# mhozza/covest

Measured on AMD Instinct MI355X. Metric: grid-point log-likelihood evals/s, repeat model, 10k-bin hist, higher is better.
Workload: dtype f64

## Files before the change

### covest_amd/csrc/ll_factored.hip

```cpp
#include <hip/hip_runtime.h>

#include <algorithm>
#include <mutex>
#include <type_traits>

#include "direct_point.h"
#include "handback.h"
#include "fastmath.h"
#include "kernels.h"
#include "point_fetch.h"
#include "streams.h"
#include "wave.h"

namespace covest {

namespace {

typedef double d4 __attribute__((ext_vector_type(4)));

constexpr double kShareScale = 0x1p128;


template <int N, int MU>
__device__ __forceinline__ void contract_step(int i, const double *cur, const int (&a_off)[MU], const int (&cut)[MU],
                                              const double (&r4)[MU], double (&wrun)[MU], d4 (&acc)[MU])
{
    double a[N];
#pragma unroll
    for (int k = 0; k < N; ++k)
        a[k] = cur[a_off[k] + 4 * i];
#pragma unroll
    for (int k = 0; k < N; ++k) {
        const double w = (i < cut[k]) ? wrun[k] : 0.0;
        wrun[k] *= r4[k];
        acc[k] = __builtin_amdgcn_mfma_f64_16x16x4f64(a[k], w, acc[k], 0, 0, 0);
    }
}

[[maybe_unused]] constexpr int kLdWide = 290;
template <int NT, int HU, bool TAIL, bool PLAIN, int LDC = 0>
__global__ __launch_bounds__(NT) void ll_factored_kernel(const DevModel m, const int32_t n_tiles, const int32_t n_items,
                                                         const double *__restrict__ tile_dbl,
                                                         const int32_t *__restrict__ tile_int,
                                                         const FactoredPlan plan,
                                                         double *__restrict__ out_ll, const SubList sub_list)
{
    const TileView tv = tile_view_from(n_tiles, n_items, tile_dbl, tile_int);
#ifdef COVEST_DIAG
    const long long dgx_0 = (long long)clock64();
    long long dgx_1 = 0, dgx_2 = 0, dgx_3 = 0, dgx_4 = 0;
#endif
    constexpr int NW = NT / kWave;
    constexpr int MU = 2 * HU;
    static_assert(MU == 6, "contract loops are written for 6 slots");
    constexpr bool SPO = PLAIN && TAIL;
    constexpr bool NEED_SCAL = !PLAIN;
    constexpr int LOG_DEG = PLAIN ? 3 : 5;
    const int LD = LDC ? LDC : plan.ld;
    constexpr int NE = FactoredLds::entries_of(NT);
    const FactoredLds lay{NT, plan.n_buf, LD, SPO};
    extern __shared__ double Gs[];
    __shared__ __attribute__((aligned(16))) double log_tab[kLogTableDoubles];
    __shared__ unsigned sub_rec[NE * 2];
    __shared__ __attribute__((aligned(16))) double2 rowc[2][kTileBins];
    __shared__ __attribute__((aligned(16))) double rows[NEED_SCAL ? 2 : 1][NEED_SCAL ? kTileBins : 2];
    __shared__ __attribute__((aligned(16))) double rho_tab[PLAIN ? NW * MU * 4 : 4];
    __shared__ double lconst_s;
    static_assert(MU == kMaxUnits, "the LDS layout counts kMaxUnits slots a wave");
    static_assert(sizeof(log_tab) + sizeof(sub_rec) + sizeof(rowc) + sizeof(rows) + sizeof(rho_tab) + sizeof(lconst_s) + 6 * 15 <=
                      kFactoredStaticLds, "the planners' LDS budget (tiles.h) must hold the kernel's static LDS");

    const int tid = threadIdx.x;
    const int lane = tid & (kWave - 1);
    const int wave = __builtin_amdgcn_readfirstlane(tid / kWave);
    const double p_clamp = plan.p_clamp;
    const double zero_frac = kZeroSteps * (kGridStep / p_clamp);
    const int list_mode = PLAIN ? 0 : plan.list_mode;

    const int n_seg = list_mode ? plan.n_seg : 1;
    const int unit = list_mode ? (int)blockIdx.x / n_seg : (int)blockIdx.x;
    const int seg = list_mode ? (int)blockIdx.x - unit * n_seg : 0;
    const int seg_items = (n_items + n_seg - 1) / n_seg;
    const int t_begin = seg * seg_items, t_end = min(n_items, t_begin + seg_items);
    const int64_t ce = (PLAIN || list_mode == 0) ? plan.ce_end - 1 - unit : plan.ce_begin + unit;
    const bool list = list_mode == 1 || list_mode == 2;
    const int64_t ic = list ? ce : ce / plan.n_e;
    const int64_t ie = list ? ce : ce - ic * plan.n_e;
    double par[kMaxParams] = {plan.c_axis[ic], plan.e_axis[ie], 0, 0, 0};
    constexpr int kLogPerThread = (kLogTableDoubles + NT - 1) / NT;
    double log_v[kLogPerThread];
#pragma unroll
    for (int u = 0; u < kLogPerThread; ++u)
        log_v[u] = kLogTable[min(tid + u * NT, kLogTableDoubles - 1)];
    const double rho_v = PLAIN ? plan.unit_rho[(int64_t)blockIdx.y * NW * MU * 4 + min(tid, NW * MU * 4 - 1)] : 0.0;
    double lc_first = 0.0;
    if (wave == NW - 1 && t_begin + lane < t_end)
        lc_first = tv.item_lconst[t_begin + lane];
#pragma unroll
    for (int u = 0; u < kLogPerThread; ++u)
        if (tid + u * NT < kLogTableDoubles)
            log_tab[tid + u * NT] = log_v[u];
    if (PLAIN && tid < NW * MU * 4)
        rho_tab[tid] = rho_v;
#pragma unroll
    for (int u = 0; u < (NE + NT - 1) / NT; ++u)
        if (tid + u * NT < NE) {
            sub_rec[2 * (tid + u * NT)] = 0xFFFFFFFFu;
            sub_rec[2 * (tid + u * NT) + 1] = 0;
        }
    clamp_point<2>(m, par);
    const bool finite = isfinite(par[0]) && isfinite(par[1]);
    const int n_pass = PLAIN ? 1 : plan.n_pass;
    if (tid < 8 * n_pass)
        Gs[lay.rates() + tid] = error_class_rate_mul(m, par[0], par[1], tid, m.n_err);
    if (wave == NW - 1) {
        double lc = 0.0 + lc_first;
        for (int t = t_begin + lane + kWave; t < t_end; t += kWave)
            lc += tv.item_lconst[t];
        lc = wave_sum(lc);
        if (lane == 0)
            lconst_s = PLAIN ? lc - kLogRawBias<kScaleBits> * tv.suf_h[0] : lc;
    }
    __syncthreads();
#ifdef COVEST_DIAG
    dgx_1 = (long long)clock64();
#endif

    const int my_pass = n_pass == 1 ? 0 : tid / plan.pass_stride;
    const int o_local = n_pass == 1 ? tid : tid - my_pass * plan.pass_stride;
    const bool wave_builds = wave * kWave < plan.n_columns;
    const int o_base = PLAIN ? 0 : list_mode == 2 ? plan.item_obase[ce] : plan.o_base;
    const int o_mine = o_base + o_local + 1;
    double lam[8];
#pragma unroll
    for (int s = 0; s < 8; ++s)
        lam[s] = Gs[lay.rates() + 8 * my_pass + s];
    double n_total = -1.0;
    if (n_pass > 1) {
        n_total = 0.0;
        for (int s = 0; s < 8 * n_pass; ++s)
            n_total += m.comb[s] * (1.0 - exp_neg_rn((double)o_mine * Gs[lay.rates() + s]));
    }
    __syncthreads();
    StreamSet<8> st;
    if (wave_builds) {
        st.template init<false>(m, lam, o_mine, finite && my_pass < n_pass && o_local < plan.max_o, log_tab,
                                log_tab, 8 * my_pass, n_total);
    } else {
        st.gone = 0u;
#pragma unroll
        for (int s = 0; s < 8; ++s) {
            st.v[s] = 0.0;
            st.x[s] = 0.0;
            st.an.set(s, 0.0, -INFINITY);
        }
    }
#ifdef COVEST_DIAG
    dgx_2 = (long long)clock64();
#endif
    const bool lane_in_row = tid < LD - 2;
    if (tid < FactoredLds::kSlack)
        Gs[lay.slack() + tid] = 0.0;
    if (tid < lay.rows()) {
        Gs[lay.pad(tid)] = 0.0;
        Gs[lay.pad(tid) + 1] = 0.0;
    }

    const int col = lane & 15;
    const int kq = lane >> 4;
    int len[MU], cont[MU], uhalf[MU], qslot[MU], cut[MU], a_off0[MU], nsh[MU];
    double r4[MU], llacc[MU];
    uint64_t dead[MU];
    unsigned off_slots = 0;
    bool newly_dead = false;
    CompSum spacc[(TAIL && !SPO) ? MU : 1];
    CompSum so = {0.0, 0.0};
    auto wave_block = [&](int w) -> int {
        if (list)
            return w >= NW - 2 ? 1 + 2 * (int)ce + (w - (NW - 2)) : 0;
        return (int)blockIdx.y * NW + w;
    };
    const int slot_base = wave_block(wave) * MU;
    int u_qt[MU], u_s0[MU], u_len[MU], u_cont[MU], u_half[MU], u_nsh[MU], u_o0[MU], u_T[MU];
#pragma unroll
    for (int k = 0; k < MU; ++k) {
        const int at = slot_base + k;
        u_qt[k] = plan.unit_tile[at];
        u_s0[k] = plan.unit_s0[at];
        u_len[k] = plan.unit_len[at];
        u_cont[k] = plan.unit_cont[at];
        u_half[k] = plan.unit_half[at];
        u_nsh[k] = PLAIN ? plan.unit_nsh[at] : 0;
        u_o0[k] = plan.unit_o0[at];
    }
#pragma unroll
    for (int k = 0; k < MU; ++k) {
        const int qt = __builtin_amdgcn_readfirstlane(u_qt[k]);
        const bool on = qt >= 0;
        const int slot = (on ? qt : 0) * 16 + col;
        qslot[k] = on ? slot : -1;
        u_T[k] = plan.q_T[slot];
        r4[k] = plan.q_r4[slot];
    }
#pragma unroll
    for (int k = 0; k < MU; ++k) {
        const bool on = qslot[k] >= 0;
        const int first_step = __builtin_amdgcn_readfirstlane(u_s0[k]);
        len[k] = __builtin_amdgcn_readfirstlane(u_len[k]);
        cont[k] = __builtin_amdgcn_readfirstlane(u_cont[k]);
        uhalf[k] = __builtin_amdgcn_readfirstlane(u_half[k]);
        nsh[k] = PLAIN ? __builtin_amdgcn_readfirstlane(u_nsh[k]) : 0;
        a_off0[k] = (16 * uhalf[k] + col) * LD + kq + 4 * first_step;
        const int t_lane = on ? u_T[k] : 0;
        const int o0 = __builtin_amdgcn_readfirstlane(u_o0[k]);
        cut[k] = ((t_lane - (o0 + kq) + 3) >> 2) - nsh[k];
        llacc[k] = 0.0;
        dead[k] = 0;
        spacc[(TAIL && !SPO) ? k : 0].hi = 0.0;
        spacc[(TAIL && !SPO) ? k : 0].lo = 0.0;
    }

    unsigned m_first = 0, m_cont = 0, m_sh = 0;
#pragma unroll
    for (int k = 0; k < MU; ++k) {
        m_first |= (qslot[k] >= 0 && !cont[k]) ? 1u << k : 0u;
        m_cont |= cont[k] ? 1u << k : 0u;
        m_sh |= nsh[k] > 0 ? 1u << k : 0u;
    }
    double wfirst[MU], wrun[MU];
    auto load_weights = [&]() {
#pragma unroll
        for (int k = 0; k < MU; ++k) {
            const double2 pw = reinterpret_cast<const double2 *>(plan.piece_w)[(int64_t)(slot_base + k) * kWave + lane];
            wfirst[k] = pw.x;
            wrun[k] = pw.y;
        }
    };
    load_weights();

    long long dg_a = 0, dg_b = 0, dg_b0 = 0, dg_c = 0, dg_w = 0, dg_t0 = 0, dg_zero = 0, dg_enter = 0, dg_first = 0;
#ifdef COVEST_DIAG
    const bool diag = plan.diag != nullptr;
#else
    constexpr bool diag = false;
#endif
    auto walk_tile = [&](auto n_tag, double *colp, double renorm, double k0) __attribute__((always_inline)) -> double {
        constexpr int N = decltype(n_tag)::value;
        if (!lane_in_row)
            return 0.0;
        double xx[8];
#pragma unroll
        for (int s = 0; s < 8; ++s) {
            double xs = st.x[s];
            if (s < N) {
                asm volatile("" : "+v"(xs));
                xx[s] = xs * xs;
            } else {
                xx[s] = 0.0;
            }
        }
        double *row = colp;
        double tsum = 0.0;
        if (SPO) {
            double kk = k0;
#pragma unroll
            for (int b = 0; b < kTileBins; b += 2) {
                double g1, g2;
                st.template step2n<N>(xx, g1, g2);
                row[0] = g1;
                row[LD] = g2;
                row += 2 * LD;
                tsum = fma(tsum, kk, g1);
                kk += 1.0;
                tsum = fma(tsum, kk, g2);
                kk += 1.0;
            }
            tsum *= renorm;
        } else {
#pragma unroll
            for (int b = 0; b < kTileBins; b += 2) {
                double g1, g2;
                st.template step2n<N>(xx, g1, g2);
                row[0] = g1;
                row[LD] = g2;
                row += 2 * LD;
            }
        }
        st.template leave_tile_n<N>(renorm);
        return tsum;
    };
    auto build_tile = [&](int t, bool seg_start, double *dst) __attribute__((always_inline)) -> double {
        if (COVEST_SKIP_PHASE(plan, 1))
            return 0.0;
        const TileRec rc = tv.rec[t];
        const double k0 = rc.k0;
        const int nb = rc.nb;
        const int n_live = st.enter_tile(k0 - 1.0, k0 + (double)(nb - 1), rc.lgam_prev, rc.lgam_last,
                                         rc.run_start != 0 || seg_start);
        if (diag) {
            const long long now__ = (long long)clock64();
            dg_enter += now__ - dg_t0;
            dg_t0 = now__;
        }
        double *colp = dst + (lane_in_row ? tid : 0);
        const double *scal = tv.scal + (int64_t)t * kTileBins;
        if (nb == kTileBins && !(SPO && rc.has_filler != 0)) {
            if (n_live > 4)
                return walk_tile(std::integral_constant<int, 8>{}, colp, rc.renorm, k0);
            if (n_live > 2)
                return walk_tile(std::integral_constant<int, 4>{}, colp, rc.renorm, k0);
            if (n_live == 2)
                return walk_tile(std::integral_constant<int, 2>{}, colp, rc.renorm, k0);
            if (n_live == 1)
                return walk_tile(std::integral_constant<int, 1>{}, colp, rc.renorm, k0);
            if (lane_in_row) {
                if (diag)
                    dg_zero += 1;
#pragma unroll
                for (int b = 0; b < kTileBins; ++b)
                    colp[b * LD] = 0.0;
            }
            return 0.0;
        }
        double tsum = 0.0;
        for (int b = 0; b < kTileBins; ++b) {
            const double g = b < nb ? st.step() : 0.0;
            if (SPO && b < nb)
                tsum = fma(g, scal[b], tsum);
            if (lane_in_row)
                colp[b * LD] = g;
        }
        st.leave_tile(rc.renorm);
        return tsum * 0x1p476;
    };
    auto sum_tile = [&](auto n_tag, const double *scal_ptr, double scal_or_k0, double renorm) __attribute__((always_inline)) -> double {
        constexpr int N = decltype(n_tag)::value;
        double xx[8];
#pragma unroll
        for (int s = 0; s < 8; ++s) {
            double xs = st.x[s];
            if (s < N) {
                asm volatile("" : "+v"(xs));
                xx[s] = xs * xs;
            } else {
                xx[s] = 0.0;
            }
        }
        double gsum = 0.0;
        if (SPO) {
            double kk = scal_or_k0;
#pragma unroll
            for (int b = 0; b < kTileBins; b += 2) {
                double g1, g2;
                st.template step2n<N>(xx, g1, g2);
                gsum = fma(gsum, kk, g1);
                kk += 1.0;
                gsum = fma(gsum, kk, g2);
                kk += 1.0;
            }
            st.template leave_tile_n<N>(renorm);
            return gsum * renorm;
        }
        const double *scal = SPO ? nullptr : scal_ptr;
#pragma unroll
        for (int half = 0; half < 2; ++half) {
            double sc[16];
#pragma unroll
            for (int b = 0; b < 16; ++b)
                sc[b] = scal[16 * half + b];
            asm volatile("" ::: "memory");
#pragma unroll
            for (int b = 0; b < 16; b += 2) {
                double g1, g2;
                st.template step2n<N>(xx, g1, g2);
                gsum = fma(g1, sc[b], gsum);
                gsum = fma(g2, sc[b + 1], gsum);
            }
        }
        st.template leave_tile_n<N>(renorm);
        return gsum * (1.0 / kBasicScale);
    };
    auto build_tile_sum = [&](int t, bool seg_start) __attribute__((always_inline)) -> double {
        const TileRec rc = tv.rec[t];
        const double k0 = rc.k0;
        const int nb = rc.nb;
        const int n_live = SPO ? st.enter_sum_tile(k0 - 1.0, k0 + (double)(nb - 1), rc.lgam_prev, rc.lgam_last,
                                                   rc.run_start != 0 || seg_start)
                               : st.enter_tile(k0 - 1.0, k0 + (double)(nb - 1), rc.lgam_prev, rc.lgam_last,
                                               rc.run_start != 0 || seg_start);
        const double *scal = tv.scal + (int64_t)t * kTileBins;
        if (nb == kTileBins && !(SPO && rc.has_filler != 0)) {
            if (n_live > 2)
                return sum_tile(std::integral_constant<int, 8>{}, scal, k0, rc.renorm);
            if (n_live == 2)
                return sum_tile(std::integral_constant<int, 2>{}, scal, k0, rc.renorm);
            if (n_live == 1)
                return sum_tile(std::integral_constant<int, 1>{}, scal, k0, rc.renorm);
            return 0.0;
        }
        double gsum = 0.0;
        for (int b = 0; b < nb; ++b)
            gsum = fma(st.step(), scal[b], gsum);
        st.leave_tile(rc.renorm);
        return SPO ? gsum * 0x1p476 : gsum * (1.0 / kBasicScale);
    };
    bool resync = false;
    auto build_item = [&](int it, bool seg_start, double *dst) __attribute__((always_inline)) {
        const int first = TAIL ? __builtin_amdgcn_readfirstlane(tv.item_first[it]) : it;
        if (TAIL && tv.item_sum[it] != 0) {
            if (COVEST_SKIP_PHASE(plan, 1))
                return;
            const int n = __builtin_amdgcn_readfirstlane(tv.item_ntiles[it]);
            if (SPO) {
                if (!seg_start) {
                    const int tl = first + n - 1;
                    const TileRec ra = tv.rec[first], rb = tv.rec[tl];
                    const double ka = ra.k0 - 1.0, kb = rb.k0 + (double)(rb.nb - 1);
                    const double lga = ra.lgam_prev, lgb = rb.lgam_last;
                    bool matters = false;
#pragma unroll
                    for (int s = 0; s < 8; ++s) {
                        if ((st.gone >> s) & 1u)
                            continue;
                        const double lx = st.an.lx(s), c = st.an.c(s);
                        const double top = fmax(fma(ka, lx, c - lga), fma(kb, lx, c - lgb));
                        matters = matters || !(top < StreamSet<8>::kSumWindowLn) || (st.x[s] >= ka - 1.0 && st.x[s] <= kb + 1.0);
                    }
                    if (!__any(matters)) {
#pragma unroll
                        for (int s = 0; s < 8; ++s)
                            st.v[s] = 0.0;
                        resync = true;
                        return;
                    }
                }
                for (int r = 0; r < n; ++r) {
                    if (st.gone == 0xFFu && !(seg_start && r == 0))
                        break;
                    so.add(build_tile_sum(first + r, (seg_start && r == 0) || resync));
                    resync = false;
                }
                return;
            }
            double *colp = dst + (lane_in_row ? tid : 0);
            for (int r = 0; r < n; ++r) {
                const double gsum = build_tile_sum(first + r, seg_start && r == 0);
                if (lane_in_row)
                    colp[r * LD] = gsum;
            }
            for (int r = n; r < kTileBins; ++r)
                if (lane_in_row)
                    colp[r * LD] = 0.0;
        } else {
            const double tsum = build_tile(first, seg_start || (SPO && resync), dst);
            resync = false;
            if (SPO)
                so.add(tsum);
        }
    };

#define STAMP(acc)                                    \
    if (diag) {                                       \
        const long long now__ = (long long)clock64(); \
        acc += now__ - dg_t0;                         \
        dg_t0 = now__;                                \
    }
    if (diag)
        dg_t0 = (long long)clock64();
#ifdef COVEST_DIAG
    dgx_3 = (long long)clock64();
#endif

    const bool dbuf = plan.n_buf == 2;
    double nxt_h = 0.0, nxt_c = 0.0, nxt_s = 0.0;
    auto fetch_rows = [&](int it) {
        if (tid < kTileBins && it < t_end) {
            const int64_t at = (int64_t)it * kTileBins + tid;
            nxt_h = tv.item_cnt[at];
            nxt_c = tv.item_iscal[at];
            if (NEED_SCAL)
                nxt_s = tv.item_scal[at];
        }
    };
    int last_item = t_end - 1;
    if (SPO)
        while (last_item > t_begin && tv.item_sum[last_item] != 0)
            --last_item;
    const bool last_first = PLAIN && t_end - t_begin >= 2 && last_item > t_begin;
    auto tile_at = [&](int p) -> int { return last_first ? (p == t_begin ? last_item : (p <= last_item ? p - 1 : p)) : p; };
    const int t_endx = t_end + (SPO ? 1 : 0);
    fetch_rows(tile_at(t_begin));
    for (int p = t_begin - (dbuf ? 1 : 0); p < t_endx; ++p) {
        const int pb = dbuf ? p + 1 : p;
        if (SPO && pb == t_end) {
            if (wave_builds && lane_in_row) {
                double *dst = Gs + lay.buf(pb) + tid;
                dst[0] = so.hi * 0x1p-540;
                dst[LD] = so.lo * 0x1p-540;
            }
        } else if (pb < t_end) {
            if (tid < kTileBins) {
                rowc[pb & 1][tid] = make_double2(nxt_h, p_clamp * nxt_c);
                if (NEED_SCAL)
                    rows[pb & 1][tid] = nxt_s;
            }
            fetch_rows(pb + 1 < t_end ? tile_at(pb + 1) : t_end);
            if (wave_builds) {
                if (last_first && pb == t_begin + 1)
                    st.gone = 0u;
                build_item(tile_at(pb), pb == t_begin || (last_first && (pb == t_begin + 1 || pb == last_item + 1)),
                           Gs + lay.buf(pb));
            }
        }
        STAMP(dg_a)
        if (!dbuf)
            __syncthreads();
        const bool sp_item = SPO && p == t_end;
        if (p >= t_begin && !(SPO && !sp_item && tv.item_sum[tile_at(p)] != 0)) {
            const int t = tile_at(p);
            const double *cur = Gs + lay.buf(p);
            d4 acc[MU];
            const d4 zero4 = (d4){0.0, 0.0, 0.0, 0.0};
            double a0[MU];
#pragma unroll
            for (int k = 0; k < MU; ++k)
                a0[k] = cur[a_off0[k]];
            if (diag) {
                double sink = 0.0;
#pragma unroll
                for (int k = 0; k < MU; ++k)
                    sink += a0[k] + wfirst[k];
                asm volatile("" ::"v"(sink));
                const long long now__ = (long long)clock64();
                dg_first += now__ - dg_t0;
                dg_t0 = now__;
            }
#pragma unroll
            for (int k = 0; k < MU; ++k) {
                if (!PLAIN || !((m_sh >> k) & 1u) || COVEST_SKIP_PHASE(plan, 8)) {
                    acc[k] = len[k] > 0 ? __builtin_amdgcn_mfma_f64_16x16x4f64(a0[k], wfirst[k], zero4, 0, 0, 0) : zero4;
                    continue;
                }
                const double rr16 = rho_tab[4 * (wave * MU + k)];
                const double2 rt = *reinterpret_cast<const double2 *>(&rho_tab[4 * (wave * MU + k) + 2]);
                const double rr4 = rt.x, rho_n = rt.y;
                const double *g1 = cur + a_off0[k];
                int nsh_k = nsh[k];
                asm volatile("" : "+s"(nsh_k));
                const int n4 = nsh_k >> 2, rem = nsh_k & 3;
                const double *top = g1 + 4 * (1 + 4 * n4);
                const double *zp = Gs + FactoredLds{NT, plan.n_buf, LD, SPO}.slack();
                double h0 = *(rem > 0 ? top : zp), h1 = *(rem > 1 ? top + 4 : zp), h2 = *(rem > 2 ? top + 8 : zp), h3 = 0.0;
                {
                    unsigned qa = (unsigned)(uintptr_t)(top - 32);
                    int gq = n4;
                    for (; gq >= 2; gq -= 2, qa -= 256) {
                        double b0, b1, b2, b3, c0, c1, c2, c3;
                        asm volatile("ds_read_b64 %0, %8 offset:128\n\tds_read_b64 %1, %8 offset:160\n\t"
                                     "ds_read_b64 %2, %8 offset:192\n\tds_read_b64 %3, %8 offset:224\n\t"
                                     "ds_read_b64 %4, %8\n\tds_read_b64 %5, %8 offset:32\n\t"
                                     "ds_read_b64 %6, %8 offset:64\n\tds_read_b64 %7, %8 offset:96\n\t"
                                     "s_waitcnt lgkmcnt(0)"
                                     : "=&v"(b0), "=&v"(b1), "=&v"(b2), "=&v"(b3), "=&v"(c0), "=&v"(c1), "=&v"(c2), "=&v"(c3)
                                     : "v"(qa));
                        h0 = fma_vvv(fma(h0, rr16, b0), rr16, c0);
                        h1 = fma_vvv(fma(h1, rr16, b1), rr16, c1);
                        h2 = fma_vvv(fma(h2, rr16, b2), rr16, c2);
                        h3 = fma_vvv(fma(h3, rr16, b3), rr16, c3);
                    }
                    if (gq > 0) {
                        double b0, b1, b2, b3;
                        asm volatile("ds_read_b64 %0, %4 offset:128\n\tds_read_b64 %1, %4 offset:160\n\t"
                                     "ds_read_b64 %2, %4 offset:192\n\tds_read_b64 %3, %4 offset:224\n\t"
                                     "s_waitcnt lgkmcnt(0)"
                                     : "=&v"(b0), "=&v"(b1), "=&v"(b2), "=&v"(b3)
                                     : "v"(qa));
                        h0 = fma_vvv(h0, rr16, b0);
                        h1 = fma_vvv(h1, rr16, b1);
                        h2 = fma_vvv(h2, rr16, b2);
                        h3 = fma_vvv(h3, rr16, b3);
                    }
                }
                const double hs = fma(fma(fma(h3, rr4, h2), rr4, h1), rr4, h0);
                acc[k] = __builtin_amdgcn_mfma_f64_16x16x4f64(hs, wrun[k] * rho_n, zero4, 0, 0, 0);
                acc[k] = __builtin_amdgcn_mfma_f64_16x16x4f64(a0[k], wfirst[k], acc[k], 0, 0, 0);
            }
            STAMP(dg_b0)
            if (!COVEST_SKIP_PHASE(plan, 2)) {
                int a_off[MU];
#pragma unroll
                for (int k = 0; k < MU; ++k)
                {
                    int nsh_k = nsh[k];
                    asm volatile("" : "+s"(nsh_k));
                    a_off[k] = a_off0[k] + 4 * nsh_k;
                }
                int i = 1;
                for (; i < len[5]; ++i)
                    contract_step<6, MU>(i, cur, a_off, cut, r4, wrun, acc);
                for (; i < len[4]; ++i)
                    contract_step<5, MU>(i, cur, a_off, cut, r4, wrun, acc);
                for (; i < len[3]; ++i)
                    contract_step<4, MU>(i, cur, a_off, cut, r4, wrun, acc);
                for (; i < len[2]; ++i)
                    contract_step<3, MU>(i, cur, a_off, cut, r4, wrun, acc);
                for (; i < len[1]; ++i)
                    contract_step<2, MU>(i, cur, a_off, cut, r4, wrun, acc);
                for (; i < len[0]; ++i)
                    contract_step<1, MU>(i, cur, a_off, cut, r4, wrun, acc);
            }
#pragma unroll
            for (int k = MU - 1; k >= 1; --k)
                if ((m_cont >> k) & 1u) {
                    asm volatile("" ::: "memory");
                    acc[k - 1] += acc[k];
                }
            STAMP(dg_b)
            const bool item_is_sum = TAIL && !SPO && tv.item_sum[t] != 0;
#pragma unroll
            for (int k = 0; k < MU; ++k) {
                if (list_mode == 2) {
                    if (qslot[k] >= 0 && !cont[k] && col == 0) {
#pragma unroll
                        for (int r = 0; r < 4; ++r)
                            plan.partial[(ce * tv.n_items + t) * kTileBins + 16 * uhalf[k] + kq + 4 * r] =
                                acc[k][r] * (rows[NEED_SCAL ? (p & 1) : 0][NEED_SCAL ? 16 * uhalf[k] + kq + 4 * r : 0] * kShareScale);
                    }
                    continue;
                }
                if (list_mode == 3) {
                    if (qslot[k] >= 0 && !cont[k]) {
                        double *row = plan.partial + (((ce - plan.ce_first) * plan.n_cols_partial + qslot[k]) * tv.n_items + t) * kTileBins +
                                      16 * uhalf[k] + kq;
#pragma unroll
                        for (int r = 0; r < 4; ++r) {
                            const double share = acc[k][r] * (rows[NEED_SCAL ? (p & 1) : 0][NEED_SCAL ? 16 * uhalf[k] + kq + 4 * r : 0] * kShareScale);
                            row[4 * r] = plan.o_base == 0 ? share : row[4 * r] + share;
                        }
                    }
                    continue;
                }
                if (SPO && sp_item) {
                    if (qslot[k] >= 0 && !cont[k] && uhalf[k] == 0 && lane < 32)
                        Gs[lay.spo_parts(t_end) + kq * NE + (wave * MU + k) * 16 + col] = acc[k][0];
                    continue;
                }
                if (TAIL && !SPO && item_is_sum) {
                    if ((m_first >> k) & 1u) {
#pragma unroll
                        for (int r = 0; r < 4; ++r)
                            spacc[k].add(acc[k][r]);
                    }
                    continue;
                }
                if (((m_first >> k) & 1u) && !COVEST_SKIP_PHASE(plan, 4)) {
                    const double2 *rc = &rowc[p & 1][16 * uhalf[k] + kq];
                    double h4[4], c4[4], x4[4], lg4[4];
#pragma unroll
                    for (int r = 0; r < 4; ++r) {
                        const double2 hc = rc[4 * r];
                        h4[r] = hc.x;
                        c4[r] = hc.y;
                    }
                    if (TAIL && !SPO) {
                        const double *sr = &rows[NEED_SCAL ? (p & 1) : 0][NEED_SCAL ? 16 * uhalf[k] + kq : 0];
#pragma unroll
                        for (int r = 0; r < 4; ++r)
                            spacc[k].add(acc[k][r] * sr[NEED_SCAL ? 4 * r : 0]);
                    }
                    uint64_t low[4];
#pragma unroll
                    for (int r = 0; r < 4; ++r)
                        low[r] = __ballot(acc[k][r] < c4[r]);
                    if (__builtin_expect(((low[0] | low[1] | low[2] | low[3]) & ~dead[k]) != 0, 0)) {
                        uint64_t subm = 0, zero = 0;
#pragma unroll
                        for (int r = 0; r < 4; ++r) {
                            const uint64_t z = __ballot(acc[k][r] <= c4[r] * zero_frac) & low[r];
                            zero |= z;
                            subm |= low[r] & ~z;
                            acc[k][r] = max_raw(acc[k][r], c4[r]);
                        }
                        const uint64_t zc = (zero | (zero >> 16) | (zero >> 32) | (zero >> 48)) & 0xFFFFull;
                        dead[k] |= zc * 0x0001000100010001ull;
                        newly_dead = newly_dead || zc != 0;
                        const uint64_t cm = (subm | (subm >> 16) | (subm >> 32) | (subm >> 48)) & 0xFFFFull;
                        if (kq == 0 && ((cm >> col) & 1)) {
                            const unsigned u = 2u * (unsigned)(TAIL ? tv.item_first[t] : t) + (unsigned)uhalf[k];
                            unsigned *rec = &sub_rec[((wave * MU + k) * 16 + col) * 2];
                            rec[0] = min(rec[0], u);
                            rec[1] = max(rec[1], u + 1);
                        }
                    }
#pragma unroll
                    for (int r = 0; r < 4; ++r)
                        x4[r] = acc[k][r];
                    fast_log_bits_n<4, LOG_DEG, kScaleBits, PLAIN>(x4, lg4, log_tab);
#pragma unroll
                    for (int r = 0; r < 4; ++r)
                        llacc[k] = fma(h4[r], lg4[r], llacc[k]);
                    __builtin_amdgcn_sched_barrier(0);
                }
            }
            load_weights();
            if (PLAIN && newly_dead) {
                newly_dead = false;
#pragma unroll
                for (int k = 0; k < MU; ++k) {
                    const bool first_dead = ((m_first >> k) & 1u) && dead[k] == ~0ull;
                    const bool piece_dead = k > 0 && ((m_cont >> k) & 1u) && ((off_slots >> (k - 1)) & 1u);
                    if (first_dead || piece_dead) {
                        off_slots |= 1u << k;
                        m_first &= ~(1u << k);
                        m_sh &= ~(1u << k);
                        len[k] = 0;
                    }
                }
            }
            STAMP(dg_c)
        }
        __syncthreads();
#ifdef COVEST_DIAG
        if (diag && (plan.skip_phases & 0x10000)) {
            const long long now__ = (long long)clock64();
            if (lane == 0) {
                const int grp = (plan.skip_phases & 0x20000) ? min(7, p - t_begin + 1)
                                                              : min(7, (p - t_begin + 1) * 8 / (t_end - t_begin + 1));
                plan.diag[((int64_t)(blockIdx.x * gridDim.y + blockIdx.y) * NW + wave) * 8 + grp] += now__ - dg_t0;
            }
        }
#endif
        STAMP(dg_w)
    }

#ifdef COVEST_DIAG
    dgx_4 = (long long)clock64();
#endif
    if (diag && lane == 0 && !(plan.skip_phases & 0x50000)) {
        long long *d = plan.diag + ((int64_t)(blockIdx.x * gridDim.y + blockIdx.y) * NW + wave) * 8;
        d[0] = dg_a;
        d[1] = dg_b;
        d[2] = dg_c;
        d[3] = dg_w;
        d[4] = dg_b0;
        d[5] = dg_zero;
        d[6] = dg_enter;
        d[7] = dg_first;
    }
#undef STAMP
    if (list_mode >= 2)
        return;
    const double lconst = lconst_s;
    constexpr int kEntries = (NE + NT - 1) / NT;
    constexpr bool kEntriesEarly = TAIL;
    int en_qt[kEntries], en_half[kEntries], en_cont[kEntries], en_pair[kEntries], en_qo[kEntries];
    auto fetch_entries = [&]() __attribute__((always_inline)) {
#pragma unroll
        for (int u = 0; u < kEntries; ++u) {
            const int e = min(tid + u * NT, NE - 1);
            const int at = wave_block(e / (MU * 16)) * MU + (e / 16) % MU;
            en_qt[u] = plan.unit_tile[at];
// ... 407 lines not shown
```

### covest_amd/csrc/plan_factored.cpp

```cpp
#include "host.h"

#include <initializer_list>

using namespace covest;

namespace covest {

double copy_number_weight_host(double q1, double q2, double q, int o)
{
    if (o == 1)
        return q1;
    if (o == 2)
        return (1 - q1) * q2;
    return (1 - q1) * (1 - q2) * q * std::pow(1 - q, (double)(o - 3));
}

namespace {

constexpr int kQTileSlots = 16;
constexpr int kStepColumns = 4;
constexpr int kStepLanes = kStepColumns * kQTileSlots;
static_assert(kStepLanes == 64, "one wave holds the weights of a step");
static_assert(2 * kHalfUnits == kMaxUnits, "a wave's slots are two halves' (tiles.h)");
constexpr int mfma_steps_of(int columns) { return (columns + kStepColumns - 1) / kStepColumns; }
// ... 210 lines not shown
    int min_shared;
};

Charges planner_charges(const covest_model *m)
{
    Charges ch = {kUnitOverhead, kBuildCost, kSharedStepsPerMfma, kLastBuilderExtra, kMinSharedSteps};
    if (m->has_tiles && m->tv.n_items > 0)
        ch.build_cost = (int)std::lround((double)(m->low_tile_share >= 0.75 ? kBuildCostLowKeys : kBuildCost) *
                                         (double)m->tv.n_tiles / (double)m->tv.n_items);
#if defined(COVEST_DIAG) || defined(COVEST_TUNE)
    if (const char *v = std::getenv("COVEST_FACTORED_UNIT_OVERHEAD"))
        ch.unit_overhead = std::atoi(v);
    if (const char *v = std::getenv("COVEST_FACTORED_BUILD_COST"))
        ch.build_cost = std::atoi(v);
    if (const char *v = std::getenv("COVEST_FACTORED_SHARED_DIV"))
        ch.shared_div = std::max(1, std::atoi(v));
    if (const char *v = std::getenv("COVEST_FACTORED_LAST_BUILDER_EXTRA"))
        ch.last_builder_extra = std::atoi(v);
    if (const char *v = std::getenv("COVEST_FACTORED_MIN_SHARED"))
        ch.min_shared = std::atoi(v);
#endif
    return ch;
}

struct Unit {
    int tile, half, cost, pieces;
};

int place_units(int blk, const PartSpec &ps, const PartColumns &pc, const PartGeometry &geo, const Charges &ch,
                std::vector<std::vector<Unit>> &held)
{
    const int nw = geo.n_waves();
    std::vector<Unit> units;
    for (int qt = blk; qt < ps.n_qtiles(); qt += geo.n_qblocks)
        for (int h = 0; h < 2; ++h) {
            const int nsh = pc.nsh[(size_t)qt];
            units.push_back({qt, h, ps.n_pass * std::max(1, pc.mfma_steps(qt)) + ch.unit_overhead +
                                        (nsh ? 1 + (nsh + ch.shared_div - 1) / ch.shared_div : 0), 1});
        }
    std::stable_sort(units.begin(), units.end(), [](const Unit &a, const Unit &b) { return a.cost > b.cost; });
    const int n_bins = std::min(4, nw);
    std::vector<long> bin_load((size_t)n_bins, 0), wave_load((size_t)nw, 0);
    if (geo.n_buf == 2)
        for (int w = 0; w < nw && w * 64 < geo.n_columns; ++w) {
            const int cost = ch.build_cost + (((w + 1) * 64 >= geo.n_columns && w >= n_bins) ? ch.last_builder_extra : 0);
            bin_load[(size_t)(w % n_bins)] += cost;
            wave_load[(size_t)w] += cost;
        }
    held.assign((size_t)nw, {});
    for (const Unit &u : units) {
        int best_wave = -1;
        for (int w = 0; w < nw; ++w) {
            if ((int)held[(size_t)w].size() >= geo.units_per_wave)
                continue;
            if (best_wave < 0) {
                best_wave = w;
                continue;
            }
            const long lb = bin_load[(size_t)(w % n_bins)], bb = bin_load[(size_t)(best_wave % n_bins)];
            if (lb < bb || (lb == bb && wave_load[(size_t)w] < wave_load[(size_t)best_wave]))
                best_wave = w;
        }
        if (best_wave < 0)
            return fail(COVEST_E_INVALID, "K-factored plan: no wave has room for a unit (internal)");
        held[(size_t)best_wave].push_back(u);
        bin_load[(size_t)(best_wave % n_bins)] += u.cost;
        wave_load[(size_t)best_wave] += u.cost;
    }
    return COVEST_OK;
}

void write_wave_slots(std::vector<Unit> &mine, size_t slot0, const PartSpec &ps, const PartColumns &pc,
                      const PartGeometry &geo, UnitTables &ut)
{
    const int n_pass = ps.n_pass;
    auto piece_len = [&](const Unit &u) { return (pc.mfma_steps(u.tile) + u.pieces - 1) / u.pieces; };
    int used = (int)mine.size() * n_pass;
    while (used + n_pass <= kMaxUnits && !mine.empty()) {
        size_t longest = 0;
        for (size_t i = 1; i < mine.size(); ++i)
            if (piece_len(mine[i]) > piece_len(mine[longest]))
                longest = i;
        if (pc.nsh[(size_t)mine[longest].tile])
            break;
        Unit trial = mine[longest];
        trial.pieces += 1;
        if (piece_len(trial) < kMinPieceSteps)
            break;
        mine[longest].pieces += 1;
        used += n_pass;
    }
    std::stable_sort(mine.begin(), mine.end(), [&](const Unit &a, const Unit &b) { return piece_len(a) > piece_len(b); });
    size_t k = 0;
    for (const Unit &u : mine) {
        bool first = true;
        for (int pass = 0; pass < n_pass; ++pass)
            for (int p = 0; p < u.pieces; ++p, ++k) {
                ut.set(slot0 + k, u.tile, u.half, pass * (geo.pass_stride / kStepColumns) + p * piece_len(u),
                       1 + kStepColumns * p * piece_len(u), piece_len(u), !first, pc.nsh[(size_t)u.tile]);
                first = false;
            }
    }
}

int deal_qblock(int blk, const PartSpec &ps, const PartColumns &pc, const PartGeometry &geo, const Charges &ch, UnitTables &ut)
{
    std::vector<std::vector<Unit>> held;
    const int rc = place_units(blk, ps, pc, geo, ch, held);
    if (rc != COVEST_OK)
        return rc;
    for (int w = 0; w < geo.n_waves(); ++w)
        write_wave_slots(held[(size_t)w], ((size_t)blk * geo.n_waves() + w) * kMaxUnits, ps, pc, geo, ut);
    return COVEST_OK;
}

void slot_weights(size_t at, const PartSpec &ps, const PartColumns &pc, const UnitTables &ut, double *piece_w, double *unit_rho)
{
    const int qt = ut.tile[at], nsh = ut.nsh[at], o0 = ut.o0[at];
    const int o_first = ps.o_base + o0;
    double pw_q = NAN, pw_geo = 0.0, pw_16 = 0.0, pw_4 = 0.0, pw_inv = 0.0, pw_after = 0.0;
    for (int colx = 0; colx < kQTileSlots; ++colx) {
        const size_t ls = (size_t)qt * kQTileSlots + (size_t)colx;
        if (pc.q_orig[ls] < 0)
            continue;
        const double q1 = pc.w[ls].q1, q2 = pc.w[ls].q2, q = pc.w[ls].q;
        const double head = (1 - q1) * (1 - q2) * q, base = 1 - q;
        if (!(q == pw_q)) {
            pw_q = q;
            pw_geo = o_first >= 3 ? std::pow(base, (double)(o_first - 3)) : 1.0;
            if (nsh > 0) {
                pw_16 = std::pow(base, 16.0);
                pw_4 = std::pow(base, 4.0);
                pw_inv = 1.0 / std::pow(base, 4.0 * (double)nsh);
                pw_after = std::pow(base, (double)(o_first + kStepColumns * (nsh + 1) - 3));
            }
        }
        double geo = pw_geo;
        for (int d = 0; d < 2 * kStepColumns; ++d) {
            const int o = o_first + d;
            double w;
            if (o < 3) {
                w = copy_number_weight_host(q1, q2, q, o);
            } else {
                w = head * geo;
                geo *= base;
            }
            if (d < kStepColumns && o0 + d >= (int)pc.q_t[ls])
                w = 0.0;
            if (d < kStepColumns || nsh == 0)
                piece_w[(at * kStepLanes + (size_t)((d % kStepColumns) * kQTileSlots + colx)) * 2 + (size_t)(d / kStepColumns)] = w;
        }
        if (nsh > 0) {
            unit_rho[4 * at] = pw_16;
            unit_rho[4 * at + 2] = pw_4;
            unit_rho[4 * at + 3] = pw_inv;
            double g2 = pw_after;
            for (int d = 0; d < kStepColumns; ++d, g2 *= base)
                piece_w[(at * kStepLanes + (size_t)(d * kQTileSlots + colx)) * 2 + 1] = head * g2;
        }
    }
}

void pair_halves(UnitTables &ut, size_t block_slots)
{
    for (size_t b0 = 0; b0 < ut.size(); b0 += block_slots) {
        const size_t b1 = b0 + block_slots;
        for (size_t at = b0; at < b1; ++at) {
            if (ut.tile[at] < 0 || ut.half[at] != 0 || ut.cont[at])
                continue;
            for (size_t at2 = b0; at2 < b1; ++at2)
                if (ut.tile[at2] == ut.tile[at] && ut.half[at2] == 1 && !ut.cont[at2]) {
                    ut.pair[at] = (int32_t)(at2 - b0);
                    break;
                }
        }
    }
}

void apply_diag_env(FactoredPlan &pl)
{
#ifdef COVEST_DIAG
    if (std::getenv("COVEST_FACTORED_NBUF"))
        pl.n_buf = std::max(1, std::min(pl.n_buf, std::atoi(std::getenv("COVEST_FACTORED_NBUF"))));
    const char *skip = std::getenv("COVEST_FACTORED_SKIP");
    pl.skip_phases = skip ? std::atoi(skip) : 0;
    if (pl.list_mode == 0 && std::getenv("COVEST_FACTORED_DIAG")) {
        void *dp = nullptr;
        const size_t bytes = (size_t)(pl.ce_end - pl.ce_begin) * pl.n_qblocks * (pl.n_threads / 64) * 8 * sizeof(long long);
        if (hipMalloc(&dp, bytes) == hipSuccess && hipMemset(dp, 0, bytes) == hipSuccess) {
            pl.diag = static_cast<long long *>(dp);
            if (std::atoi(std::getenv("COVEST_FACTORED_DIAG")) >= 2)
                pl.skip_phases |= 0x10000;
            if (std::atoi(std::getenv("COVEST_FACTORED_DIAG")) == 3)
                pl.skip_phases |= 0x20000;
            if (std::atoi(std::getenv("COVEST_FACTORED_DIAG")) == 4)
                pl.skip_phases = (pl.skip_phases & ~0x10000) | 0x40000;
            std::fprintf(stderr, "COVEST_FACTORED_DIAG %p %zu\n", dp, bytes);
        }
    }
#else
    (void)pl;
#endif
}

int build_plan_part(covest_grid *g, const double *const *axes, const std::vector<int32_t> &t_table, const QOrder &qo,
                    const PartSpec &ps, const Charges &ch, DevBuf &buf, FactoredPlan &pl, std::vector<int32_t> *q_orig_out)
{
    const covest_model *m = g->model;
    const PartColumns pc = part_columns(m, axes, t_table, qo, ps);
    if (q_orig_out)
        *q_orig_out = pc.q_orig;
    const PartGeometry geo =
        part_geometry(pc.t_loc_max, ps.n_pass, ps.n_qtiles(), std::max<int64_t>(1, g->len[0] * g->len[1]));
    UnitTables ut(geo.n_unit());
    for (int blk = 0; blk < geo.n_qblocks; ++blk) {
        const int rc = deal_qblock(blk, ps, pc, geo, ch, ut);
        if (rc != COVEST_OK)
            return rc;
    }
    std::vector<double> piece_w(ut.size() * kStepLanes * 2, 0.0), unit_rho(ut.size() * 4, 1.0);
    for (size_t at = 0; at < ut.size(); ++at)
        if (ut.tile[at] >= 0)
            slot_weights(at, ps, pc, ut, piece_w.data(), unit_rho.data());
    pair_halves(ut, geo.block_slots());
    PlanPack pack({{PlanPack::QR4, &pc.r4}, {PlanPack::PieceW, &piece_w}, {PlanPack::UnitRho, &unit_rho}},
                  {{PlanPack::QT, &pc.q_t}, {PlanPack::QOrig, &pc.q_orig}, {PlanPack::UnitTile, &ut.tile},
                   {PlanPack::UnitHalf, &ut.half}, {PlanPack::UnitS0, &ut.s0}, {PlanPack::UnitO0, &ut.o0},
                   {PlanPack::UnitLen, &ut.len}, {PlanPack::UnitCont, &ut.cont}, {PlanPack::UnitNsh, &ut.nsh},
                   {PlanPack::UnitPair, &ut.pair}});
    const int rc = upload_to_grid(g, buf, pack);
    if (rc != COVEST_OK)
        return rc;
    fill_plan(pl, geo, ps.n_pass, pack);
    pl.c_axis = g->src.axis[0];
    pl.e_axis = g->src.axis[1];
    pl.n_e = g->len[1];
    pl.n_q = qo.nq;
    pl.ce_begin = g->flat_begin / qo.nq;
    pl.ce_end = (g->flat_end + qo.nq - 1) / qo.nq;
    pl.n_qtiles = ps.n_qtiles();
    pl.o_base = ps.o_base;
    pl.flat_begin = g->flat_begin;
    pl.flat_end = g->flat_end;
    pl.list_mode = ps.list_mode;
    pl.p_clamp = clamp_for(m, qo.t_max);
    pl.ce_first = pl.ce_begin;
    pl.n_cols_partial = (int64_t)ps.n_qtiles() * kQTileSlots;
    apply_diag_env(pl);
    return COVEST_OK;
}

struct ByThreshold {
    const std::vector<int32_t> &t_table;
    bool operator()(int32_t a, int32_t b) const { return t_table[(size_t)a] > t_table[(size_t)b]; }
};

bool wants_shared_order(const QOrder &qo, int n_pass)
{
    const int64_t group = qo.n1 * qo.n2, group_padded = (group + kQTileSlots - 1) / kQTileSlots * kQTileSlots;
    bool share = n_pass == 1 && 3 * (group_padded - group) <= group;
#ifdef COVEST_DIAG
    if (const char *share_env = std::getenv("COVEST_FACTORED_SHARE"))
        share = share && std::atoi(share_env) != 0;
#endif
    return share;
}

QOrder plain_order(QOrder qo, const std::vector<int32_t> &t_table)
{
    std::vector<int32_t> all((size_t)qo.nq);
    for (int64_t i = 0; i < qo.nq; ++i)
        all[(size_t)i] = (int32_t)i;
    std::stable_sort(all.begin(), all.end(), ByThreshold{t_table});
    qo.n_qtiles = (int32_t)((qo.nq + kQTileSlots - 1) / kQTileSlots);
    qo.order.assign((size_t)qo.n_qtiles * kQTileSlots, -1);
    std::copy(all.begin(), all.end(), qo.order.begin());
    qo.tile_nsh.assign((size_t)qo.n_qtiles, 0);
    return qo;
}

QOrder shared_order(QOrder qo, const std::vector<int32_t> &t_table, int chunk, int min_shared)
{
    struct Tile {
        int32_t slot[kQTileSlots];
        int t_hi, t_lo;
    };
    const int64_t group = qo.n1 * qo.n2;
    std::vector<Tile> tiles;
    std::vector<int32_t> one((size_t)group);
    for (int64_t c = 0; c < qo.n3; ++c) {
        for (int64_t ab = 0; ab < group; ++ab)
            one[(size_t)ab] = (int32_t)(ab * qo.n3 + c);
        std::stable_sort(one.begin(), one.end(), ByThreshold{t_table});
        for (int64_t at = 0; at < group; at += kQTileSlots) {
            Tile t;
            const int64_t live = std::min<int64_t>(kQTileSlots, group - at);
            for (int64_t i = 0; i < kQTileSlots; ++i)
                t.slot[i] = i < live ? one[(size_t)(at + i)] : -1;
            t.t_hi = (int)t_table[(size_t)t.slot[0]];
            t.t_lo = (int)t_table[(size_t)t.slot[live - 1]];
            tiles.push_back(t);
        }
    }
    std::stable_sort(tiles.begin(), tiles.end(), [](const Tile &a, const Tile &b) { return a.t_hi > b.t_hi; });
    qo.n_qtiles = (int32_t)tiles.size();
    qo.order.resize(tiles.size() * kQTileSlots);
// ... 217 lines not shown
```

### covest_amd/csrc/tiles.h

```cpp
#pragma once
#include <hip/hip_runtime_api.h>
#include <stdint.h>

namespace covest {

constexpr int kTileBins = 32;
constexpr int kScaleBits = 540;
constexpr double kScaleLn = 540.0 * 0.693147180559945309417232121458;
constexpr double kWindowLn = -760.0;
constexpr int kBasicShift = 64;
constexpr double kBasicScale = 0x1p64;

struct alignas(64) TileRec {
    double k0, lgam_prev, lgam_last, renorm;
    int32_t nb, run_start, all_zero, has_filler;
    double pad[2];
};
static_assert(sizeof(TileRec) == 64, "one cache line");

struct TileView {
    int32_t n_tiles;
    int32_t n_items;
    const double *dbl_base;
    const int32_t *int_base;
    const double *first_key;
    const int32_t *n_bins;
    const int32_t *run_start;
    const int32_t *all_zero;
    const int32_t *has_filler;
    const double *lgam_prev;
    const double *lgam_last;
    const double *renorm;
    const double *scal;
    const double *cnt;
    const double *item_cnt;
    const double *item_scal;
    const double *item_iscal;
    const double *item_lconst;
    const double *suf_h;
    const double *suf_jh;
    const double *suf_lgh;
    const double *suf_first;
    const double *suf_first_lg;
    const double *last_key;
    const int32_t *item_first;
    const int32_t *item_ntiles;
    const int32_t *item_sum;
    const int32_t *row_bin;
    const TileRec *rec;
};

inline __host__ __device__ int64_t tile_arrays_dbl(int32_t nt, int32_t ni)
{
    const int64_t n = 4 * (int64_t)nt + 2 * (int64_t)nt * kTileBins + 3 * (int64_t)ni * kTileBins + ni + 5 * ((int64_t)nt + 1) + 2;
    return (n + 7) / 8 * 8;
}
inline __host__ __device__ int64_t tile_dbl_count(int32_t nt, int32_t ni) { return tile_arrays_dbl(nt, ni) + 8 * (int64_t)nt; }
inline __host__ __device__ int64_t tile_int_count(int32_t nt, int32_t ni) { return 4 * (int64_t)nt + 3 * (int64_t)ni + (int64_t)nt * kTileBins; }

inline __host__ __device__ TileView tile_view_from(int32_t nt, int32_t ni, const double *dbl, const int32_t *ints)
{
    TileView tv;
    tv.n_tiles = nt;
    tv.n_items = ni;
    tv.dbl_base = dbl;
    tv.int_base = ints;
    tv.first_key = dbl;
    tv.lgam_prev = dbl + nt;
    tv.lgam_last = dbl + 2 * (int64_t)nt;
    tv.renorm = dbl + 3 * (int64_t)nt;
    tv.scal = dbl + 4 * (int64_t)nt;
    tv.cnt = tv.scal + (int64_t)nt * kTileBins;
    tv.item_cnt = tv.cnt + (int64_t)nt * kTileBins;
    tv.item_scal = tv.item_cnt + (int64_t)ni * kTileBins;
    tv.item_iscal = tv.item_scal + (int64_t)ni * kTileBins;
    tv.item_lconst = tv.item_iscal + (int64_t)ni * kTileBins;
    tv.suf_h = tv.item_lconst + ni;
    tv.suf_jh = tv.suf_h + (nt + 1);
    tv.suf_lgh = tv.suf_jh + (nt + 1);
    tv.suf_first = tv.suf_lgh + (nt + 1);
    tv.suf_first_lg = tv.suf_first + (nt + 1);
    tv.last_key = tv.suf_first_lg + (nt + 1);
    tv.n_bins = ints;
    tv.run_start = ints + nt;
    tv.all_zero = ints + 2 * (int64_t)nt;
    tv.has_filler = ints + 3 * (int64_t)nt;
    tv.item_first = ints + 4 * (int64_t)nt;
    tv.item_ntiles = tv.item_first + ni;
    tv.item_sum = tv.item_ntiles + ni;
    tv.row_bin = tv.item_sum + ni;
    tv.rec = reinterpret_cast<const TileRec *>(dbl + tile_arrays_dbl(nt, ni));
    return tv;
}

constexpr int kMaxUnits = 6;
constexpr int kHalfUnits = 3;
constexpr int kBuildCost = 18;
constexpr int kBuildCostLowKeys = 24;
constexpr int kLowKeyTile = 384;
#ifndef COVEST_LIST_SEGMENTS
#define COVEST_LIST_SEGMENTS 16
#endif
constexpr int kListSegments = COVEST_LIST_SEGMENTS;
constexpr int kMinPieceSteps = 6;
constexpr int kSharedStepsPerMfma = 4;
constexpr int kMinSharedSteps = 3;
constexpr int kLastBuilderExtra = 4;
constexpr int kUnitOverhead = 2;

struct FactoredPlan {
    const double *c_axis, *e_axis;
    int64_t n_e;
    int64_t ce_begin, ce_end;
    int64_t n_q;
    int32_t n_qtiles;
    int32_t max_o;
    int32_t n_pass;
    int32_t pass_stride;
    int32_t n_columns;
    int32_t o_base;
    int32_t n_threads;
    int32_t half_units;
    int32_t n_qblocks;
    int32_t ld;
    int32_t n_buf;
    const int32_t *unit_tile;
    const int32_t *unit_half;
    const int32_t *unit_s0;
    const int32_t *unit_o0;
    const int32_t *unit_len;
    const int32_t *unit_cont;
    const int32_t *unit_nsh;
    const int32_t *unit_pair;
    const double *unit_rho;
    const double *piece_w;
    const int32_t *qtile_nsteps;
    const int32_t *qtile_nfull;
    const int32_t *q_T;
    const int32_t *q_orig;
    const double *q_first8;
    const double *q_r4;
    int64_t flat_begin, flat_end;
    int32_t list_mode;
    double p_clamp;
    int32_t n_seg;
    const int32_t *item_obase;
    double *partial;
    int64_t ce_first;
    int64_t n_cols_partial;
    long long *diag;
    int32_t skip_phases;
};

constexpr int kLdsBytes = 160 * 1024;
constexpr int kFactoredStaticLds = 13440;

constexpr __host__ __device__ int factored_ld(int columns) { return (columns + kTileBins - 1) / kTileBins * kTileBins + 2; }

struct FactoredLds {
    int nt, n_buf, ld;
    bool spo;
    static constexpr int kSlack = 64;
    static constexpr int kRates = 32;
    __host__ __device__ static constexpr int entries_of(int nt) { return nt / 64 * kMaxUnits * 16; }
    __host__ __device__ constexpr int entries() const { return entries_of(nt); }
    __host__ __device__ constexpr int rows() const { return n_buf * kTileBins; }
    __host__ __device__ constexpr int buf(int b) const { return n_buf == 2 ? (b & 1) * kTileBins * ld : 0; }
    __host__ __device__ constexpr int pad(int row) const { return row * ld + ld - 2; }
    __host__ __device__ constexpr int slack() const { return n_buf * kTileBins * ld; }
    __host__ __device__ constexpr int rates() const { return 0; }
    __host__ __device__ constexpr bool spo_inside() const
    {
        return kTileBins * ld >= (n_buf == 2 ? 0 : 2 * ld) + 3 * entries();
    }
    __host__ __device__ constexpr int spo_parts(int t_end) const
    {
        return !spo_inside() ? slack() + kSlack : n_buf == 2 ? buf(t_end + 1) + entries() : 2 * ld + entries();
    }
    __host__ __device__ constexpr int part_ll() const { return 0; }
    __host__ __device__ constexpr int part_hi(int t_end) const { return spo ? spo_parts(t_end) : entries(); }
    __host__ __device__ constexpr int part_lo(int t_end) const { return part_hi(t_end) + entries(); }
    __host__ __device__ constexpr int total() const
    {
        const int a = slack() + kSlack, b = 3 * entries(), c = spo && !spo_inside() ? slack() + kSlack + 2 * entries() : 0;
        return a > b ? (a > c ? a : c) : (b > c ? b : c);
    }
    __host__ __device__ constexpr bool fits() const { return total() * (int)sizeof(double) + kFactoredStaticLds <= kLdsBytes; }
};

constexpr __host__ __device__ int factored_n_buf(int ld) { return FactoredLds{512, 2, ld, true}.fits() ? 2 : 1; }

#ifdef COVEST_DIAG
#define COVEST_SKIP_PHASE(plan, bits) (((plan).skip_phases & (bits)) != 0)
#else
#define COVEST_SKIP_PHASE(plan, bits) false
#endif

}
```

Baseline: 413.6 million.

## Truncate shared and contract steps beyond a per-tile negligible-probability band

Adds a band computation that, per wave and tile, uses Newton iterations on a log-domain bound to find the step past which remaining terms fall below a fixed log threshold (e^-56). The shared-step and contract loops are then clipped to that band, skipping MFMA work whose contribution is negligible. The planner now stores ln(base) in unit_rho for this bound, and the build cost constant is raised to shift planning toward configurations that benefit. This adds per-wave setup math and a readlane per item, and it risks accuracy if the bound is not conservative.

```diff
diff --git a/covest_amd/csrc/band.h b/covest_amd/csrc/band.h
--- /dev/null
+++ b/covest_amd/csrc/band.h
@@ -0,0 +1,83 @@
+#pragma once
+#include <math.h>
+
+#ifndef COVEST_HD
+#ifdef __HIPCC__
+#define COVEST_HD __host__ __device__
+#else
+#define COVEST_HD
+#endif
+#endif
+
+namespace covest {
+
+constexpr double kBandLn = 56.0;
+constexpr int kBandClasses = 8;
+constexpr int kBandNewton = 2;
+
+constexpr int kBandMinShared = 8;
+
+struct Band {
+    int step_lo, step_hi;
+};
+
+struct BandTile {
+    double key_first, key_last, cls_first, cls_last;
+};
+
+COVEST_HD inline BandTile band_tile(const double *ln_rate, const double *ln_comb, double key_first, double key_last)
+{
+    BandTile t = {key_first, key_last, -INFINITY, -INFINITY};
+    for (int s = 1; s < kBandClasses; ++s) {
+        const double lc = ln_comb[s] - ln_comb[0], lr = ln_rate[s] - ln_rate[0];
+        if (!(lc > -INFINITY))
+            continue;
+        const double a = lc + key_first * lr, b = lc + key_last * lr;
+        t.cls_first = a > t.cls_first ? a : t.cls_first;
+        t.cls_last = b > t.cls_last ? b : t.cls_last;
+    }
+    return t;
+}
+
+struct BandMathHost {
+    double ln(double x) const { return log(x); }
+    double rcp(double x) const { return 1.0 / x; }
+};
+
+template <class Math>
+COVEST_HD inline Band band_of_unit(const Math &mth, double rate0, double ln_1mq, int o_ref_max, int n_steps, const BandTile &t)
+{
+    const Band full = {0, n_steps};
+    const double mu = -ln_1mq, L = rate0 + mu;
+    if (!(rate0 > 0.0) || !(mu >= 0.0) || !(L < 1e300) || !(t.key_first >= 1.0) || !(t.key_last >= t.key_first) ||
+        !(t.key_last < 16384.0) || o_ref_max < 3 || n_steps < 2)
+        return full;
+    const double mode = t.key_last * mth.rcp(L);
+    double o_ref = floor(mode);
+    o_ref = o_ref < 3.0 ? 3.0 : o_ref;
+    o_ref = o_ref > (double)o_ref_max ? (double)o_ref_max : o_ref;
+    const double inv_ref = mth.rcp(o_ref);
+    double a = 2.0 * mode + 8.0;
+    for (int it = 0; it < kBandNewton; ++it) {
+        const double g = -(a - o_ref) * L + t.key_last * mth.ln(a * inv_ref) + kBandLn;
+        const double dg = -L + t.key_last * mth.rcp(a);
+        if (!(dg < 0.0))
+            return full;
+        a -= g * mth.rcp(dg);
+        if (!(a > mode))
+            return full;
+    }
+    const double o_edge = ceil(a) + 1.0;
+    if (!(o_edge < 4.0 * (double)n_steps))
+        return full;
+    const int step_hi = ((int)o_edge + 2) >> 2;
+    if (step_hi < 1 || step_hi >= n_steps)
+        return full;
+    const double o_drop = 1.0 + 4.0 * (double)step_hi, o_top = 4.0 * (double)n_steps;
+    const double base = o_ref * rate0 - (o_drop - o_ref) * mu + kBandLn, ln_o = mth.ln(o_top * inv_ref);
+    if (!(base + t.key_first * ln_o + t.cls_first <= 0.0) || !(base + t.key_last * ln_o + t.cls_last <= 0.0))
+        return full;
+    return Band{0, step_hi};
+}
+
+}
diff --git a/covest_amd/csrc/ll_factored.hip b/covest_amd/csrc/ll_factored.hip
--- a/covest_amd/csrc/ll_factored.hip
+++ b/covest_amd/csrc/ll_factored.hip
@@ -4,6 +4,7 @@
 #include <mutex>
 #include <type_traits>
 
+#include "band.h"
 #include "direct_point.h"
 #include "handback.h"
 #include "fastmath.h"
@@ -66,9 +67,10 @@
     __shared__ __attribute__((aligned(16))) double rows[NEED_SCAL ? 2 : 1][NEED_SCAL ? kTileBins : 2];
     __shared__ __attribute__((aligned(16))) double rho_tab[PLAIN ? NW * MU * 4 : 4];
     __shared__ double lconst_s;
+    __shared__ double band_ln[PLAIN ? kBandClasses : 1];
     static_assert(MU == kMaxUnits, "the LDS layout counts kMaxUnits slots a wave");
-    static_assert(sizeof(log_tab) + sizeof(sub_rec) + sizeof(rowc) + sizeof(rows) + sizeof(rho_tab) + sizeof(lconst_s) + 6 * 15 <=
-                      kFactoredStaticLds, "the planners' LDS budget (tiles.h) must hold the kernel's static LDS");
+    static_assert(sizeof(log_tab) + sizeof(sub_rec) + sizeof(rowc) + sizeof(rows) + sizeof(rho_tab) + sizeof(lconst_s) +
+                          sizeof(band_ln) + 7 * 15 <= kFactoredStaticLds, "the planners' LDS budget (tiles.h) must hold the kernel's static LDS");
 
     const int tid = threadIdx.x;
     const int lane = tid & (kWave - 1);
@@ -135,6 +137,8 @@
 #pragma unroll
     for (int s = 0; s < 8; ++s)
         lam[s] = Gs[lay.rates() + 8 * my_pass + s];
+    if (PLAIN && tid < kBandClasses)
+        band_ln[tid] = fast_log(Gs[lay.rates() + tid], log_tab);
     double n_total = -1.0;
     if (n_pass > 1) {
         n_total = 0.0;
@@ -226,6 +230,37 @@
         m_first |= (qslot[k] >= 0 && !cont[k]) ? 1u << k : 0u;
         m_cont |= cont[k] ? 1u << k : 0u;
         m_sh |= nsh[k] > 0 ? 1u << k : 0u;
+    }
+    unsigned band_w0 = ~0u, band_w1 = ~0u;
+    bool wave_bands = false;
+#pragma unroll
+    for (int k = 0; k < MU; ++k)
+        wave_bands = wave_bands || (PLAIN && !wave_builds && nsh[k] >= kBandMinShared);
+    if (PLAIN && wave_bands) {
+        struct {
+            const double *tab;
+            __device__ double ln(double x) const { return fast_log(x, tab); }
+            __device__ double rcp(double x) const
+            {
+                const double r = __builtin_amdgcn_rcp(x);
+                return fma(fma(-x, r, 1.0), r, r);
+            }
+        } const mth = {log_tab};
+        const int it = min(lane, t_end - 1);
+        const double key_first = tv.rec[TAIL ? tv.item_first[it] : it].k0;
+        const double key_last = (lane < kWave - 1 ? key_first : tv.rec[n_tiles - 1].k0) + (double)(kTileBins - 1);
+        const BandTile bt = band_tile(band_ln, m.ln_comb, key_first, key_last);
+#pragma unroll
+        for (int k = 0; k < MU; ++k) {
+            if (nsh[k] < kBandMinShared)
+                continue;
+            const Band b = band_of_unit(mth, lam[0], rho_tab[4 * (wave * MU + k) + 1], 4 + 4 * nsh[k], nsh[k] + len[k], bt);
+            const unsigned hi = (unsigned)min(b.step_hi, 255);
+            if (k < 4)
+                band_w0 = (band_w0 & ~(255u << (8 * k))) | (hi << (8 * k));
+            else
+                band_w1 = (band_w1 & ~(255u << (8 * (k - 4)))) | (hi << (8 * (k - 4)));
+        }
     }
     double wfirst[MU], wrun[MU];
     auto load_weights = [&]() {
@@ -525,6 +560,13 @@
 #pragma unroll
             for (int k = 0; k < MU; ++k)
                 a0[k] = cur[a_off0[k]];
+            unsigned bw0 = ~0u, bw1 = ~0u;
+            if (PLAIN && !sp_item) {
+                const int bl = min(__builtin_amdgcn_readfirstlane(t), kWave - 1);
+                bw0 = (unsigned)__builtin_amdgcn_readlane((int)band_w0, bl);
+                bw1 = (unsigned)__builtin_amdgcn_readlane((int)band_w1, bl);
+            }
+            auto band_hi = [&](int k) -> int { return (int)(((k < 4 ? bw0 >> (8 * k) : bw1 >> (8 * (k - 4)))) & 255u); };
             if (diag) {
                 double sink = 0.0;
 #pragma unroll
@@ -547,6 +589,8 @@
                 const double *g1 = cur + a_off0[k];
                 int nsh_k = nsh[k];
                 asm volatile("" : "+s"(nsh_k));
+                if (PLAIN)
+                    nsh_k = min(nsh_k, band_hi(k) - 1);
                 const int n4 = nsh_k >> 2, rem = nsh_k & 3;
                 const double *top = g1 + 4 * (1 + 4 * n4);
                 const double *zp = Gs + FactoredLds{NT, plan.n_buf, LD, SPO}.slack();
@@ -588,25 +632,27 @@
             STAMP(dg_b0)
             if (!COVEST_SKIP_PHASE(plan, 2)) {
                 int a_off[MU];
+                int lenb[MU];
 #pragma unroll
                 for (int k = 0; k < MU; ++k)
                 {
                     int nsh_k = nsh[k];
                     asm volatile("" : "+s"(nsh_k));
                     a_off[k] = a_off0[k] + 4 * nsh_k;
+                    lenb[k] = PLAIN ? min(len[k], max(band_hi(k) - nsh_k, 1)) : len[k];
                 }
                 int i = 1;
-                for (; i < len[5]; ++i)
+                for (; i < lenb[5]; ++i)
                     contract_step<6, MU>(i, cur, a_off, cut, r4, wrun, acc);
-                for (; i < len[4]; ++i)
+                for (; i < lenb[4]; ++i)
                     contract_step<5, MU>(i, cur, a_off, cut, r4, wrun, acc);
-                for (; i < len[3]; ++i)
+                for (; i < lenb[3]; ++i)
                     contract_step<4, MU>(i, cur, a_off, cut, r4, wrun, acc);
-                for (; i < len[2]; ++i)
+                for (; i < lenb[2]; ++i)
                     contract_step<3, MU>(i, cur, a_off, cut, r4, wrun, acc);
-                for (; i < len[1]; ++i)
+                for (; i < lenb[1]; ++i)
                     contract_step<2, MU>(i, cur, a_off, cut, r4, wrun, acc);
-                for (; i < len[0]; ++i)
+                for (; i < lenb[0]; ++i)
                     contract_step<1, MU>(i, cur, a_off, cut, r4, wrun, acc);
             }
 #pragma unroll
diff --git a/covest_amd/csrc/plan_factored.cpp b/covest_amd/csrc/plan_factored.cpp
--- a/covest_amd/csrc/plan_factored.cpp
+++ b/covest_amd/csrc/plan_factored.cpp
@@ -386,6 +386,7 @@
         }
         if (nsh > 0) {
             unit_rho[4 * at] = pw_16;
+            unit_rho[4 * at + 1] = std::log(base);
             unit_rho[4 * at + 2] = pw_4;
             unit_rho[4 * at + 3] = pw_inv;
             double g2 = pw_after;
diff --git a/covest_amd/csrc/tiles.h b/covest_amd/csrc/tiles.h
--- a/covest_amd/csrc/tiles.h
+++ b/covest_amd/csrc/tiles.h
@@ -95,7 +95,7 @@
 
 constexpr int kMaxUnits = 6;
 constexpr int kHalfUnits = 3;
-constexpr int kBuildCost = 18;
+constexpr int kBuildCost = 27;
 constexpr int kBuildCostLowKeys = 24;
 constexpr int kLowKeyTile = 384;
 #ifndef COVEST_LIST_SEGMENTS
```

After: 438.9 million, median of 6. 1.06x the previous value.
